# c-f-h/pyiga

Hardware: AMD Instinct MI355X
Metric: assembled elements/sec (3D p=4, 128^3 spans) + HBM-roofline %; 1/2/4/8 GPU (higher is better)
Workload: dtype f64

## Files before the change

### pyiga_amd/csrc/fused3.hip

```cpp
#include "igx_internal.h"
#include "fused_common.h"
#include <algorithm>
#include <cstdio>
#include <cstdlib>
#include <cstring>
#include <vector>

#ifndef BF3_FIXED_PASS
#define BF3_FIXED_PASS 1
#endif
#ifndef BF3_MASS_AXSYM
#define BF3_MASS_AXSYM 1
#endif
#ifndef BF3_MASS_STW
#define BF3_MASS_STW 1
#endif
#ifndef BF3_MASS_STW_QMAX
#define BF3_MASS_STW_QMAX 3
#endif

namespace igx {

template <int P1, int P2, int Q, int NLG, int NRO, int NCW, int SYM> struct BF3Geom {
    static constexpr int P1_ = P1, P2_ = P2, Q_ = Q;
    static constexpr int p1 = P1 - 1, p2 = P2 - 1, W1 = 2 * P1 - 1, W2 = 2 * P2 - 1, TL = 64 * NLG;
    static constexpr int NSET = SYM == 2 ? 2 : 1;
    static constexpr int QS = Q + (Q % 2 == 0 ? 1 : 0), NSP = (TL + Q - 1) / Q;
    static constexpr int TLP = TL + NSP * (QS - Q);
    static constexpr int VS = Q * P2 * 2 + ((Q * P2 * 2) % 4 == 2 ? 0 : 2), NV2 = NSP * VS;
    static constexpr int LS = NRO * TLP + 2;
    static constexpr int NRING = p1 * (p1 + 1) / 2 + p1;
    static constexpr int NRL = NRING + P1;
    static constexpr int T0 = p2 * (p2 + 1) / 2;
    static constexpr int NEL = 2 * p2 * W2;
    static constexpr int off_sets() { return (W1 * LS + 1) & ~1; }
    static constexpr int off_v2(int R) { return (off_sets() + NSET * (NRL * R * W2 + 2) + 1) & ~1; }
    static constexpr int off_etab(int R) { return off_v2(R) + NV2; }
    static constexpr int lds_doubles(int R) { return off_etab(R) + NEL * 2; }
    static constexpr int rmax()
    {
        int R = TL / Q - p2;
        while (R > 1 && lds_doubles(R) * 8 > 160 * 1024) --R;
        return R;
    }
    static constexpr int RMAX = rmax();
    static constexpr int RW = RMAX * W2;
    static constexpr int SETSZ = NRL * RW + 2;
    static constexpr int OFF_PAD = NRL * RW;
    static constexpr int roff(int d) { return RW * ((d - 1) * (d + 2) / 2); }
    static constexpr int OFF_CUR = NRING * RW;
    static constexpr int OFF_SETS = off_sets(), OFF_V2 = off_v2(RMAX), OFF_ETAB = off_etab(RMAX);
    static constexpr int LDS_BYTES = lds_doubles(RMAX) * 8;
    static constexpr int NSUB = (RW + 63) / 64;
    static constexpr int npc(int pl) { return (RMAX + pl - p2 - 1) / (pl - p2); }
    static constexpr int npass(int pl) { return (W1 * npc(pl) + 64 / pl - 1) / (64 / pl); }
    static constexpr int pick()
    {
        int best = 64;
        const int cand[4] = {64, 32, 21, 16};
        for (int i = 1; i < 4; ++i)
            if (cand[i] > 2 * p2 && npass(cand[i]) < npass(best)) best = cand[i];
        return best;
    }
    static constexpr int PL = pick(), PPP = 64 / PL, NPC = npc(PL), RP = PL - p2;
};

struct BF3Blk {
    int i0, j0, diag0, c0i, c0j, cj0, ci0, rlo, rhi, row_lo, nrows, stD, stT, ne;
    long long S12;
};

typedef int bf3_v4i __attribute__((ext_vector_type(4)));

template <class Gm> struct BF3Row {
    int on, l0, c1, rp1d, sub1, sub2, sub3, sub4, sub5;
    __device__ __forceinline__ static BF3Row of(const BFArgs &A, const BF3Blk &B, const int t)
    {
        cip rp1 = (cip)A.rp1, jlo1 = (cip)A.jlo1, jhi1 = (cip)A.jhi1;
        constexpr int p1 = Gm::p1, RW = Gm::RW;
        BF3Row r;
        const int d = t - 1;
        r.on = d >= B.rlo && d < B.rhi;
        const int dc = min(max(d, 0), A.N1 - 1);
        const int jl1 = jlo1[dc];
        r.c1 = jhi1[dc] - jl1; r.l0 = p1 - (dc - jl1);
        r.rp1d = rp1[dc];
        r.sub1 = Gm::roff(1) + (int)((unsigned)dc % 2u) * RW; r.sub2 = Gm::roff(2) + (int)((unsigned)dc % 3u) * RW;
        r.sub3 = Gm::roff(3) + (int)((unsigned)dc % 4u) * RW; r.sub4 = Gm::roff(4) + (int)((unsigned)dc % 5u) * RW;
        r.sub5 = Gm::roff(5) + (int)((unsigned)dc % 6u) * RW;
        return r;
    }
    __device__ __forceinline__ int line_off(const int l) const
    {
        constexpr int p1 = Gm::p1;
        int o = Gm::OFF_CUR + (l - p1) * Gm::RW;
        o = l == p1 - 1 ? sub1 : o;
        if (p1 >= 2) o = l == p1 - 2 ? sub2 : o;
        if (p1 >= 3) o = l == p1 - 3 ? sub3 : o;
        if (p1 >= 4) o = l == p1 - 4 ? sub4 : o;
        if (p1 >= 5) o = l == p1 - 5 ? sub5 : o;
        return o;
    }
    __device__ __forceinline__ bool line_ok(const int l) const { return l < Gm::W1 && l >= l0 && l - l0 < c1; }
};
__device__ __forceinline__ __amdgpu_buffer_rsrc_t bf3_rs(double *ptr, const int len) { return __builtin_amdgcn_make_buffer_rsrc((void *)ptr, (short)0, len, 0x00020000); }

// ... 27 lines not shown
            return;
        }
        const long long shift = (long long)W2 * B.row_lo - Gm::T0;
        const long long lenD = ((long long)B.c0i * B.S12 - shift) * 8, lenT = ((long long)B.c0j * B.S12 - shift) * 8;
        pD = A.data + ((long long)rp0[B.i0] * B.S12 - A.nnz_off + shift); nD = B.stD ? (int)lenD : 0;
        pT = A.data + ((long long)rp0[B.j0] * B.S12 - A.nnz_off + shift); nT = B.stT ? (int)lenT : 0;
        const int c0min = min(B.c0i, B.c0j);
        inv = (int)(max(lenD, lenT) / (8 * max(c0min * 2 - 1, 1))) + 1;
#pragma unroll
        for (int c = 0; c < NSUB; ++c) {
            const int q = c * 64 + lane, rr = q / W2, i2 = B.row_lo + rr;
            const bool ok = q < RW && rr < B.nrows && i2 >= p2 && i2 <= A.N2 - 1 - p2;
            rrv[c] = ok ? W2 * i2 - Gm::T0 : inv;
        }
    }
    __device__ __forceinline__ static int line_of(const int sw, const int c, const int j) { return (int)((unsigned)(sw + ROT * c) % (unsigned)NS) + NS * j; }

    template <int X>
    __device__ __forceinline__ void move_row(double *sets, double *dump, const int sw, const int lane, const Row &r, double *ptr, const int len, const int sK, const int soff0)
    {
        int lb_ = lane, lc_ = lanec;
        asm volatile("" : "+v"(lb_), "+v"(lc_));
        double *bs = sets + X * Gm::SETSZ + lb_, *bc = sets + X * Gm::SETSZ + (NSUB - 1) * 64 + lc_;
        double v[NST];
#pragma unroll
        for (int c = 0; c < NSUB; ++c)
#pragma unroll
            for (int j = 0; j < JMAX; ++j) {
                const int l = line_of(sw, c, j);
                double *src = (c == NSUB - 1 ? bc : bs + c * 64) + r.line_off(min(l, W1 - 1));
// ... 29 lines not shown
            const int sD = 8 * B.c0i * (int)A.S1, sT = 8 * B.c0j * (int)A.S1;
            const int oD = 8 * (W2 * (B.c0i * r.rp1d + B.cj0 * r.c1) - r.l0), oT = 8 * (W2 * (B.c0j * r.rp1d + B.ci0 * r.c1) - r.l0);
            move_row<0>(sets, dump, sw, lane, r, pD, r.on ? nD : 0, sD, oD);
            if (NSET == 2) move_row<1>(sets, dump, sw, lane, r, pT, r.on ? nT : 0, sT, oT);
            if (SYM == 3) move_row<0>(sets, dump, sw, lane, r, pT, r.on ? nT : 0, sT, oT);
            return;
        }
        move_row<0>(sets, dump, sw, lane, r, pD, r.on ? nD : 0, 8 * (B.c0i * r.c1 - 1), 8 * ((int)((long long)B.c0i * A.S2) * r.rp1d + W2 * (B.cj0 * r.c1 - r.l0)));
        if (NSET == 2)
            move_row<1>(sets, dump, sw, lane, r, pT, r.on ? nT : 0, 8 * (B.c0j * r.c1 - 1), 8 * ((int)((long long)B.c0j * A.S2) * r.rp1d + W2 * (B.ci0 * r.c1 - r.l0)));
        if (SYM == 3)
            move_row<0>(sets, dump, sw, lane, r, pT, r.on ? nT : 0, 8 * (B.c0j * r.c1 - 1), 8 * ((int)((long long)B.c0j * A.S2) * r.rp1d + W2 * (B.ci0 * r.c1 - r.l0)));
    }
};

template <int NR, int NLG, int NQ> struct BF3DenseSplit {
    static constexpr int NA = (NR - 2) * NLG, NB = NLG;
    static constexpr int ka() { if (NA == 0) return 0; int k = 1; while (NA * k + NB * ((3 * k + 1) / 2) < NQ) ++k; return k; }
    static constexpr int KA = ka(), KB = NA == 0 ? (NQ + NB - 1) / NB : (3 * KA + 1) / 2;
    static constexpr int QB = NA * KA < NQ ? NA * KA : NQ;
};
constexpr int BF3_FAR = 0x7f000000;
template <class Gm, int NH, int SYM, int K, int QLO, int QHI, int QSTR, bool TR>
struct BF3StoreDense {
    static constexpr int p1 = Gm::p1, p2 = Gm::p2, W1 = Gm::W1, W2 = Gm::W2, WW = W1 * W2, RW = Gm::RW, NSET = SYM == 2 ? 2 : 1;
    using Row = BF3Row<Gm>;
    double svD[K], svT[NSET == 2 ? K : 1];
    int pk[K];
    int lane8;
    double *pD, *pT;
    long long nD, nT;

    __device__ __forceinline__ void init(const BFArgs &A, const BF3Blk &B, const int sw, const int lane)
    {
        cip rp0 = (cip)A.rp0;
        lane8 = lane * 8;
        pD = A.data + ((long long)rp0[B.i0] * B.S12 - A.nnz_off); nD = B.stD ? (long long)B.c0i * B.S12 * 8 : 0;
        pT = A.data + ((long long)rp0[B.j0] * B.S12 - A.nnz_off); nT = B.stT ? (long long)B.c0j * B.S12 * 8 : 0;
#pragma unroll
        for (int k = 0; k < K; ++k) {
            svD[k] = 0.0;
            if (NSET == 2) svT[k] = 0.0;
            const int qi = QLO + sw + QSTR * k;
            const int q = qi * 64 + lane, rr = q / WW, rem = q - rr * WW, l = rem / W2, e = rem - l * W2, i2 = B.row_lo + rr;
            const bool ok = qi < QHI && q < Gm::RMAX * WW && rr < B.nrows && i2 >= p2 && i2 <= A.N2 - 1 - p2;
            pk[k] = ok ? (4 * l) | ((rr * W2 + e) << 6) | (rr << 18) : (int)(0x80000000u | 60u);
        }
// ... 68 lines not shown
        const int lane = lane8 >> 3;
        const int offl = (unsigned)(lane - r.l0) < (unsigned)r.c1 ? 0 : BF3_FAR;
#pragma unroll
        for (int k = 0; k < K; ++k) {
            int pkk = pk[k];
            asm volatile("" : "+v"(pkk));
            const int rr = (pkk >> 18) & 0xff;
            const int q8 = __builtin_amdgcn_ds_bpermute(pkk & 60, offl) + ((QLO + sw + QSTR * k) * 512 + lane8);
            bf2_buffer_store(dD, (int)__mul24(rr, dlD) + q8, 0, svD[k]);
            if (NSET == 2) bf2_buffer_store(dT, (int)__mul24(rr, dlT) + q8, 0, svT[k]);
            if (SYM == 3) bf2_buffer_store(dT, (int)__mul24(rr, dlT) + q8, 0, svD[k]);
        }
    }
};

template <class Gm, int NCW, int NH, int SYM, bool TR>
__device__ __forceinline__ void bf3_edge_rows(const BFArgs &A, const BF3Blk &B, double *sets, const bf3_v4i *etab, const int t, const int cw, const int lane)
{
    constexpr int W1 = Gm::W1, W2 = Gm::W2;
    if (B.ne == 0) return;
    cip rp0 = (cip)A.rp0;
    const BF3Row<Gm> r = BF3Row<Gm>::of(A, B, t);
    const long long shift = (long long)W2 * B.row_lo - Gm::T0;
    static_assert(SYM != 3 || NH == 1, "per-axis symmetry: the second store reads the rows again (no halves, no clears)");
#pragma unroll
    for (int X = 0; X < (SYM == 3 ? 2 : Gm::NSET); ++X) {
        if (X == 0 ? !B.stD : !B.stT) continue;
        const int c0x = X == 0 ? B.c0i : B.c0j, cx = X == 0 ? B.cj0 : B.ci0;
        double *px = A.data + ((long long)rp0[X == 0 ? B.i0 : B.j0] * B.S12 - A.nnz_off + (TR ? 0 : shift));
        const int nx = (int)(((long long)c0x * B.S12 - (TR ? 0 : shift)) * 8);
        const unsigned sA = TR ? (unsigned)(c0x * r.rp1d + cx * r.c1) : (unsigned)(c0x * r.c1);
        const unsigned sC = (unsigned)(8 * c0x * (int)A.S1);
        const int soffr = TR ? 0 : 8 * (int)((long long)c0x * A.S2) * r.rp1d;
        for (int l = (int)((unsigned)(cw + NCW - X) % (unsigned)NCW); l < W1; l += NCW) {
            const unsigned sB = TR ? (unsigned)r.c1 : (unsigned)max(cx * r.c1 + l - r.l0, 0);
            const __amdgpu_buffer_rsrc_t dsc = bf3_rs(px, (r.on && r.line_ok(l)) ? nx : 0);
            double *lb = sets + (SYM == 3 ? 0 : X) * Gm::SETSZ + r.line_off(l);
            for (int ch = 0; ch * 64 < B.ne * W2; ++ch) {
                const bf3_v4i e = etab[min(ch * 64 + lane, Gm::NEL - 1)];
// ... 8 lines not shown
            }
        }
    }
}

struct BF3SweepCtx { const BF3Blk *B; double *sets, *dump; int sw, tlp; };
template <int P1, int Q, int D, int MASK, int RI, int NA, int NLG, class StoreT, bool STW, bool MULT>
__device__ __forceinline__ void bf3_sweeper(const BFArgs &A, const int r0, const int g2l, const int g2, const int s_begin, const int t_sw, const int d_begin,
                                            const int rhi, double *lines, const int LS, const BF3SweepCtx &sc)
{
    constexpr BFRole R = bf_role(MASK, RI);
    constexpr int p1 = P1 - 1;
    constexpr bool ST = STW && (RI >= 1 || bf_nroles(MASK) == 1);
    const int slane = threadIdx.x & 63;
    StoreT store;
    if constexpr (ST) store.init(A, *sc.B, sc.sw, slane);
    BF_STAMP_DECL
    __builtin_amdgcn_s_setprio(BF2_PRIO_S);
    cdp V1 = (cdp)A.V1;
    cip fa1 = (cip)A.fa1;
    double acc[P1][P1];
#pragma unroll
    for (int a = 0; a < P1; ++a)
#pragma unroll
        for (int b = 0; b < P1; ++b) acc[a][b] = 0.0;
    __amdgpu_buffer_rsrc_t rsrc[4][NA];
    int urs[4][NA];
    const int voff = g2 * 8;
#pragma unroll
    for (int t1 = 0; t1 < 4; ++t1)
#pragma unroll
// ... 142 lines not shown
            else bf3_sweeper<P1, Q, D, MASK, RI, NA, NLG, StoreA, STW, MULT>(A, r0, g2l, g2, s_begin, t_sw, d_begin, rhi, lines, LS, sc);
        } else BF3SweepDispatch<P1, Q, D, MASK, NA, NLG, StoreA, StoreB, STW, MULT, RI + 1>::run(A, role, r0, g2l, g2, s_begin, t_sw, d_begin, rhi, lines, LS, sc);
    }
};
template <int P1, int Q, int D, int MASK, int NA, int NLG, class StoreA, class StoreB, bool STW, bool MULT, int RI>
struct BF3SweepDispatch<P1, Q, D, MASK, NA, NLG, StoreA, StoreB, STW, MULT, RI, true> {
    __device__ static __forceinline__ void run(const BFArgs &, int, int, int, int, int, int, int, int, double *, int, const BF3SweepCtx &) {}
};

struct BF3Unit {
    const double *lines, *V2s;
    double *sets;
    int dd, rlo, rhi, nhi, row_lo, nrows, lane, npieces;
    int diag0, stD, stT;
    int rbs1, rbs2, rbs3, rbs4, rbs5;
};
template <class Gm, int NY, int MASK, int SYM, int H>
__device__ __forceinline__ void bf3_unit(const BF3Unit U, const int pass)
{
    constexpr int P2 = Gm::P2_, Q = Gm::Q_, p1 = Gm::p1, p2 = Gm::p2, W1 = Gm::W1, W2 = Gm::W2;
    constexpr int TL = Gm::TL, LS = Gm::LS, RW = Gm::RW, PL = Gm::PL, PPP = Gm::PPP, NPC = Gm::NPC, RP = Gm::RP;
    constexpr int AH = (P2 + 1) / 2;
    constexpr int A0 = H == 2 ? AH : 0, A1 = H == 1 ? AH : P2;
    const int lane = U.lane, dd = U.dd;
    int ln_ = min(lane, PPP * PL - 1);
    asm volatile("" : "+v"(ln_));
    const int ps = ln_ / PL, x = ln_ - ps * PL;
    const int pid = pass * PPP + ps;
    const int k9 = pid / NPC, pj = pid - k9 * NPC;
    const int s1 = pj * RP + x;
// ... 9 lines not shown
        for (int a = 0; a < A1 - A0; ++a)
#pragma unroll
            for (int b = 0; b < P2; ++b) { loc[a][b] = k0 + v0 * (a + 3 * b); asm volatile("" : "+v"(loc[a][b])); }
    }
#else
    bf_element<P2, NY, MASK, A0, A1, Q>(loc, kl, vl, Gm::TLP);
#endif
    const int r3 = s1 - p2;
    const bool item = lane < PPP * PL && pid < U.npieces && x >= p2 && r3 < U.nrows && la < U.nhi;
    const int oshv = max(p2 - (U.row_lo + r3), 0);
    int rb = U.rbs1;
    if (p1 >= 2) rb = la == 2 ? U.rbs2 : rb;
    if (p1 >= 3) rb = la == 3 ? U.rbs3 : rb;
    if (p1 >= 4) rb = la == 4 ? U.rbs4 : rb;
    if (p1 >= 5) rb = la == 5 ? U.rbs5 : rb;
    const int cb = Gm::OFF_CUR + la * RW;
    if (U.stD) {
        double out[W2];
#pragma unroll
        for (int a = A0; a < A1; ++a)
#pragma unroll
            for (int b = 0; b < P2; ++b) {
                if (a == 0) out[b + p2] = loc[0][b];
                else if (a == A0 || b == 0) out[b - a + p2] = bf2_from_lane(((lane - a) & 63) * 4, loc[a - A0][b]);
                else out[b - a + p2] += bf2_from_lane(((lane - a) & 63) * 4, loc[a - A0][b]);
            }
        if (item && row1 >= U.rlo && row1 < U.rhi) {
            double *dste = U.sets + ((colt && la > 0) ? rb : cb) + r3 * W2 - oshv;
            constexpr int OLO = H == 0 ? 0 : p2 - (A1 - 1), OHI = H == 0 ? 2 * p2 : 2 * p2 - A0;
            if (SYM != 0 && U.diag0) {
                const int omax = la == 0 ? p2 : 2 * p2;
#pragma unroll
                for (int o = OLO; o <= OHI; ++o)
                    if (o >= oshv && o <= omax) {
                        if (H == 0) dste[o] = out[o];
                        else (void)__hip_atomic_fetch_add(dste + o, out[o], __ATOMIC_RELAXED, __HIP_MEMORY_SCOPE_WORKGROUP);
                    }
            } else if (H == 0) {
                if (U.row_lo >= p2) {
#pragma unroll
                    for (int o = 0; o < W2; ++o) dste[o] = out[o];
                } else {
#pragma unroll
// ... 15 lines not shown
                            else (void)__hip_atomic_fetch_add(dste + o, out[o], __ATOMIC_RELAXED, __HIP_MEMORY_SCOPE_WORKGROUP);
                        }
                }
            }
        }
    }
    __builtin_amdgcn_sched_barrier(0);
#pragma unroll
    for (int a = 0; a < A1 - A0; ++a)
#pragma unroll
        for (int b = 0; b < P2; ++b) asm volatile("" : "+v"(loc[a][b]));
    __builtin_amdgcn_sched_barrier(0);
#ifdef BF3_NOT
    if (SYM != 0 && U.diag0 && U.stD) {
#else
    if (SYM != 0 && (U.diag0 ? U.stD : U.stT)) {
#endif
        double outT[W2];
#pragma unroll
        for (int b = 0; b < P2; ++b)
#pragma unroll
            for (int a = A0; a < A1; ++a) {
                if (b == 0) outT[a + p2] = loc[a - A0][0];
                else if (a == A0) outT[a + p2 - b] = bf2_from_lane(((lane - b) & 63) * 4, loc[0][b]);
                else outT[a + p2 - b] += bf2_from_lane(((lane - b) & 63) * 4, loc[a - A0][b]);
            }
        if (item && col1 >= U.rlo && col1 < U.rhi) {
            constexpr int ELO = H == 0 ? 0 : A0, EHI = H == 0 ? 2 * p2 : A1 - 1 + p2;
            if (U.diag0) {
                double *dste = U.sets + cb + r3 * W2 - oshv;
                const int emin = la == 0 ? p2 + 1 : oshv;
#pragma unroll
                for (int e = ELO; e <= EHI; ++e)
                    if (e >= emin) {
                        if (H == 0) dste[e] = outT[e];
                        else (void)__hip_atomic_fetch_add(dste + e, outT[e], __ATOMIC_RELAXED, __HIP_MEMORY_SCOPE_WORKGROUP);
                    }
            } else {
                double *dste = U.sets + Gm::SETSZ + (colt ? cb : rb) + r3 * W2 - oshv;
                if (H == 0) {
                    if (U.row_lo >= p2) {
#pragma unroll
                        for (int e = 0; e < W2; ++e) dste[e] = outT[e];
                    } else {
#pragma unroll
                        for (int e = 0; e < W2; ++e)
                            if (e >= oshv) dste[e] = outT[e];
                    }
                } else if (U.row_lo >= p2) {
#pragma unroll
                    for (int e = ELO; e <= EHI; ++e) {
                        if ((H == 1 && e < AH) || (H == 2 && e >= p2 + AH)) dste[e] = outT[e];
                        else (void)__hip_atomic_fetch_add(dste + e, outT[e], __ATOMIC_RELAXED, __HIP_MEMORY_SCOPE_WORKGROUP);
// ... 60 lines not shown
        V2s[sp * Gm::VS + (idx - sp * (Q * P2 * 2))] = (gpt >= 0 && gpt < A.G2) ? A.V2[(long long)win0 * P2 * 2 + idx] : 0.0;
    }
    if (NH >= 2)
        for (int idx = threadIdx.x; idx < Gm::OFF_V2 - Gm::OFF_SETS; idx += blockDim.x) sets[idx] = 0.0;
    const int lo_n = max(0, min(row_hi, min(p2, A.N2)) - row_lo);
    const int hi_s = max(max(p2, A.N2 - p2), row_lo), hi_n = max(0, row_hi - hi_s);
    const int ne = lo_n + hi_n;
    if (threadIdx.x < Gm::NEL) {
        const int k = threadIdx.x / W2, e = threadIdx.x - k * W2;
        bf3_v4i v; v.x = 0; v.y = 0; v.z = 0; v.w = BF2_OOB;
        if (k < ne) {
            const int i2 = k < lo_n ? row_lo + k : hi_s + (k - lo_n);
            const int jl2 = max(i2 - p2, 0), c2 = min(i2 + p2, A.N2 - 1) + 1 - jl2;
            if (e < c2) {
                const int shift = W2 * row_lo - Gm::T0;
                v.x = (i2 - row_lo) * W2 + e; v.y = 8 * A.rp2[i2]; v.z = 8 * c2; v.w = 8 * (e - shift);
                if constexpr (TR) { v.y = 8 * c2; v.z = 8 * e; v.w = A.rp2[i2]; }
            }
        }
        etab[threadIdx.x] = v;
    }

    int task = wave;
    if (NR == 4 && NLG == 2 && NCW == 8) {
        constexpr int tmap[16] = {0, 1, 2, 3, 6, 7, 4, 5, 8, 9, 10, 11, 12, 13, 14, 15};
        task = tmap[wave & 15];
    } else if (NR == 4 && NLG == 3 && NCW == 4) {
        constexpr int tmap[16] = {12, 13, 14, 15, 9, 3, 0, 2, 10, 4, 1, 7, 11, 6, 5, 8};
        task = tmap[wave & 15];
    } else if (NR == 4 && NLG == 2 && NCW == 4) {
        const int sd = wave & 3, k = wave >> 2;
        if (sd < 3) task = k == 0 ? NSW + sd : 2 * (sd + 1) + (k - 1);
        else task = k < 2 ? k : NSW + 3;
    }
    BF3Blk B;
    B.i0 = i0; B.j0 = j0; B.diag0 = diag0; B.c0i = jhi0[i0] - jlo0[i0]; B.c0j = jhi0[j0] - jlo0[j0];
    B.cj0 = j0 - jlo0[i0]; B.ci0 = i0 - jlo0[j0]; B.rlo = rlo; B.rhi = rhi;
    B.row_lo = row_lo; B.nrows = nrows; B.S12 = A.S1 * A.S2; B.ne = ne;
    B.stD = (i0 >= A.own_lo && i0 < A.own_hi) ? 1 : 0;
    B.stT = ((SYM == 2 || SYM == 3) && !diag0 && j0 >= A.own_lo && j0 < A.own_hi) ? 1 : 0;
    constexpr bool STW = NR >= 2 || (SYM == 3 && BF3_MASS_STW && Q <= BF3_MASS_STW_QMAX);
    constexpr int NQ = (Gm::RMAX * W1 * W2 + 63) / 64;
    using Split = BF3DenseSplit<NR < 2 ? 2 : NR, NLG, NQ>;
    using StoreA = BF3StoreDense<Gm, NH, SYM, Split::KA < 1 ? 1 : Split::KA, 0, Split::QB, Split::NA < 1 ? 1 : Split::NA, TR>;
    using StoreB = BF3StoreDense<Gm, NH, SYM, Split::KB, Split::QB, NQ, Split::NB, TR>;
    using StoreC = BF3Store<Gm, NCW, 1, NH, SYM, TR>;
    double *dump = lines + NR * Gm::TLP;
    if (task < NSW) {
        const int role = task / NLG, lg = task % NLG;
        const int g2l = lg * 64 + lane;
        const int g2 = min(max(win0 + g2l, 0), A.G2 - 1);
        const BF3SweepCtx sc{&B, sets, dump, role == NR - 1 ? lg : (role - 1) * NLG + lg, Gm::TLP};
        BF3SweepDispatch<P1, Q, (NH == 3 ? Q / 2 : Q), MASK, NA, NLG, StoreA, StoreB, STW, MULT, 0>::run(A, role, r0, g2l + (g2l / Q) * (Gm::QS - Q), g2, s_begin, t_sw, d_begin, rhi, lines, LS, sc);
        return;
    }

    const int cw = task - NSW;
    BF_STAMP_DECL
    __builtin_amdgcn_s_setprio(BF2_PRIO_C);
    StoreC store;
// ... 1 lines not shown
    const bool cdiag = diag0 || SYM == 3;
    const int nlines = cdiag ? P1 : W1;
    const int npieces = nlines * NPC;
    for (int t = d_begin; t < rhi + 1; ++t) {
        bar_lds();
        const int dd = t - 1;
        BF_SEG_BEGIN();
        if (dd >= d_begin && dd < rhi) {
            BF3Unit U;
            U.lines = lines; U.V2s = V2s; U.sets = sets; U.dd = dd; U.rlo = rlo; U.rhi = rhi; U.row_lo = row_lo; U.nrows = nrows;
            U.nhi = jhi1[dd] - dd;
            U.lane = lane; U.npieces = npieces; U.diag0 = cdiag; U.stD = SYM == 3 ? (B.stD | B.stT) : B.stD; U.stT = B.stT;
            U.rbs1 = Gm::roff(1) + (int)((unsigned)(dd + 1) % 2u) * RW; U.rbs2 = Gm::roff(2) + (int)((unsigned)(dd + 2) % 3u) * RW;
            U.rbs3 = Gm::roff(3) + (int)((unsigned)(dd + 3) % 4u) * RW; U.rbs4 = Gm::roff(4) + (int)((unsigned)(dd + 4) % 5u) * RW;
            U.rbs5 = Gm::roff(5) + (int)((unsigned)(dd + 5) % 6u) * RW;
            const int npass = (npieces + PPP - 1) / PPP;
            const int wslot = (int)((unsigned)(cw + t) % (unsigned)NCW);
            if constexpr (NH == 3) {
                for (int u = wslot; u < 2 * npass; u += NCW) {
                    if (u < npass) bf3_unit<Gm, NY, MASK, SYM, 2>(U, u);
                    else bf3_unit<Gm, NY, MASK, SYM, 1>(U, u - npass);
                }
            } else if (NH == 1 || npass <= NCW) {
                for (int pass = BF3_FIXED_PASS ? cw : wslot; pass < npass; pass += NCW) bf3_unit<Gm, NY, MASK, SYM, 0>(U, pass);
            } else if (BF3_FIXED_PASS && 2 * (npass - NCW) == NCW) {
                bf3_unit<Gm, NY, MASK, SYM, 0>(U, cw);
                if ((cw ^ t) & 1) bf3_unit<Gm, NY, MASK, SYM, 1>(U, NCW + (cw >> 1));
                else bf3_unit<Gm, NY, MASK, SYM, 2>(U, NCW + (cw >> 1));
            } else {
                bf3_unit<Gm, NY, MASK, SYM, 0>(U, wslot);
// ... 30 lines not shown

bool fused3_tr_fits(int p0, int p1, int p2, long long S_mid, long long S_last)
{
    const long long c0max = 2 * p0 + 1, W2 = 2 * p2 + 1;
    (void)p1;
    return 8 * W2 * c0max * S_mid < (1LL << 23) && 2 * S_last + 1 < (1LL << 24) && (2 * S_last + 1) * 8 * c0max * S_mid + 8 * W2 * 16 < (1LL << 32);
}

template <int P1, int P2, int Q, int NY, int MASK, int NA, int NLG, int NCW, int NH, int SYM, bool MULT, bool TR = false>
static int launch_bf3_k(hipStream_t st, const BFArgs &A0, int ncu_ctx)
{
    using Gm = BF3Geom<P1, P2, Q, NLG, bf_nroles(MASK), NCW, SYM>;
    constexpr size_t lds = (size_t)Gm::LDS_BYTES;
    static_assert(lds <= 160 * 1024, "k_bf3: LDS");
    static_assert(Gm::RMAX >= 1 && Gm::RMAX <= 255 && Gm::RW < 4096, "k_bf3: packed slot constants");
    static_assert((bf_nroles(MASK) * NLG + NCW) * 64 <= 1024, "k_bf3: block size");
    static_assert(NCW == 4 || NCW == 8, "k_bf3: contractor waves");
    static_assert(Gm::NSUB * 512 <= 4096, "k_bf3: immediate offsets of the stores");
    static_assert(Gm::NEL <= 1024 && Gm::W1 <= 15, "k_bf3: edge table / line index");
    constexpr int nthreads = (bf_nroles(MASK) * NLG + NCW) * 64;
    const void *fn = (const void *)k_bf3<P1, P2, Q, NY, MASK, NA, NLG, NCW, NH, SYM, MULT, TR>;
    IGX_HIP(hipFuncSetAttribute(fn, hipFuncAttributeMaxDynamicSharedMemorySize, (int)lds));
    int per_cu = 1, ncu = ncu_ctx;
    {
        int occ = 0;
        if (hipOccupancyMaxActiveBlocksPerMultiprocessor(&occ, fn, nthreads, lds) == hipSuccess && occ >= 1) per_cu = occ;
        if (ncu < 1) ncu = 256;
    }
    BFArgs A = A0;
    A.ntiles = (A.N2 + Gm::RMAX - 1) / Gm::RMAX;
// ... 183 lines not shown
```

Baseline: 173.3 million.

## Use a single shared ring set for symmetric off-diagonal blocks in 3D fused assembly

For the SYM==2 path, the kernel now keeps one LDS ring buffer with a wider row stride (2*P2 slots per row) and extra backward rings, in place of two separate ring sets for the block and its transpose. The transposed image is read from the same buffer by new store logic (BF3StoreOne) that uses packed slot indices and ds_bpermute line lookup. A second edge table covers the transposed edge rows. This cuts LDS footprint and the duplicate transpose writes by contractors, which may permit a larger row tile. The cost is more complex indexing, extra ring slots and store-side gather work.

Measured after the change: 164.3 million. 5.2% lower.

```diff
diff --git a/pyiga_amd/csrc/fused3.hip b/pyiga_amd/csrc/fused3.hip
--- a/pyiga_amd/csrc/fused3.hip
+++ b/pyiga_amd/csrc/fused3.hip
@@ -4,6 +4,7 @@
 #include <cstdio>
 #include <cstdlib>
 #include <cstring>
+#include <type_traits>
 #include <vector>
 
 #ifndef BF3_FIXED_PASS
@@ -25,6 +26,8 @@
     static constexpr int P1_ = P1, P2_ = P2, Q_ = Q;
     static constexpr int p1 = P1 - 1, p2 = P2 - 1, W1 = 2 * P1 - 1, W2 = 2 * P2 - 1, TL = 64 * NLG;
     static constexpr int NSET = SYM == 2 ? 2 : 1;
+    static constexpr bool ONE = SYM == 2;
+    static constexpr int EP = ONE ? 2 * P2 : 2 * P2 - 1;
     static constexpr int QS = Q + (Q % 2 == 0 ? 1 : 0), NSP = (TL + Q - 1) / Q;
     static constexpr int TLP = TL + NSP * (QS - Q);
     static constexpr int VS = Q * P2 * 2 + ((Q * P2 * 2) % 4 == 2 ? 0 : 2), NV2 = NSP * VS;
@@ -44,13 +47,19 @@
         return R;
     }
     static constexpr int RMAX = rmax();
-    static constexpr int RW = RMAX * W2;
-    static constexpr int SETSZ = NRL * RW + 2;
-    static constexpr int OFF_PAD = NRL * RW;
+    static constexpr int RW = RMAX * EP;
+    static constexpr int NRL1 = ONE ? 2 * NRING + p1 + 2 : NRL;
+    static constexpr int SETSZ = NRL1 * RW + 2;
+    static constexpr int OFF_PAD = NRL1 * RW;
     static constexpr int roff(int d) { return RW * ((d - 1) * (d + 2) / 2); }
     static constexpr int OFF_CUR = NRING * RW;
-    static constexpr int OFF_SETS = off_sets(), OFF_V2 = off_v2(RMAX), OFF_ETAB = off_etab(RMAX);
-    static constexpr int LDS_BYTES = lds_doubles(RMAX) * 8;
+    static constexpr int OFF_B = (NRING + 2) * RW;
+    static constexpr int roffB(int d) { return OFF_B + RW * ((d - 1) * (d + 4) / 2); }
+    static constexpr int RT = RMAX + 2 * p2;
+    static constexpr int OFF_SETS = off_sets();
+    static constexpr int OFF_V2 = ONE ? (OFF_SETS + SETSZ + 1) & ~1 : off_v2(RMAX);
+    static constexpr int OFF_ETAB = OFF_V2 + NV2;
+    static constexpr int LDS_BYTES = (OFF_ETAB + (ONE ? 2 : 1) * NEL * 2) * 8;
     static constexpr int NSUB = (RW + 63) / 64;
     static constexpr int npc(int pl) { return (RMAX + pl - p2 - 1) / (pl - p2); }
     static constexpr int npass(int pl) { return (W1 * npc(pl) + 64 / pl - 1) / (64 / pl); }
@@ -67,6 +76,7 @@
 
 struct BF3Blk {
     int i0, j0, diag0, c0i, c0j, cj0, ci0, rlo, rhi, row_lo, nrows, stD, stT, ne;
+    int neT;
     long long S12;
 };
 
@@ -74,6 +84,8 @@
 
 template <class Gm> struct BF3Row {
     int on, l0, c1, rp1d, sub1, sub2, sub3, sub4, sub5;
+    int sup1, sup2, sup3, sup4, sup5, cur, curo;
+    int sbb1, sbb2, sbb3, sbb4, sbb5, spb1, spb2, spb3, spb4, spb5;
     __device__ __forceinline__ static BF3Row of(const BFArgs &A, const BF3Blk &B, const int t)
     {
         cip rp1 = (cip)A.rp1, jlo1 = (cip)A.jlo1, jhi1 = (cip)A.jhi1;
@@ -88,8 +100,42 @@
         r.sub1 = Gm::roff(1) + (int)((unsigned)dc % 2u) * RW; r.sub2 = Gm::roff(2) + (int)((unsigned)dc % 3u) * RW;
         r.sub3 = Gm::roff(3) + (int)((unsigned)dc % 4u) * RW; r.sub4 = Gm::roff(4) + (int)((unsigned)dc % 5u) * RW;
         r.sub5 = Gm::roff(5) + (int)((unsigned)dc % 6u) * RW;
+        if constexpr (Gm::ONE) {
+            r.sup1 = Gm::roff(1) + (int)((unsigned)(dc + 1) % 2u) * RW; r.sup2 = Gm::roff(2) + (int)((unsigned)(dc + 2) % 3u) * RW;
+            r.sup3 = Gm::roff(3) + (int)((unsigned)(dc + 3) % 4u) * RW; r.sup4 = Gm::roff(4) + (int)((unsigned)(dc + 4) % 5u) * RW;
+            r.sup5 = Gm::roff(5) + (int)((unsigned)(dc + 5) % 6u) * RW;
+            r.cur = Gm::OFF_CUR + (dc & 1) * RW; r.curo = Gm::OFF_CUR + ((dc & 1) ^ 1) * RW;
+            r.sbb1 = Gm::roffB(1) + (int)((unsigned)dc % 3u) * RW; r.sbb2 = Gm::roffB(2) + (int)((unsigned)dc % 4u) * RW;
+            r.sbb3 = Gm::roffB(3) + (int)((unsigned)dc % 5u) * RW; r.sbb4 = Gm::roffB(4) + (int)((unsigned)dc % 6u) * RW;
+            r.sbb5 = Gm::roffB(5) + (int)((unsigned)dc % 7u) * RW;
+            r.spb1 = Gm::roffB(1) + (int)((unsigned)(dc + 1) % 3u) * RW; r.spb2 = Gm::roffB(2) + (int)((unsigned)(dc + 2) % 4u) * RW;
+            r.spb3 = Gm::roffB(3) + (int)((unsigned)(dc + 3) % 5u) * RW; r.spb4 = Gm::roffB(4) + (int)((unsigned)(dc + 4) % 6u) * RW;
+            r.spb5 = Gm::roffB(5) + (int)((unsigned)(dc + 5) % 7u) * RW;
+        }
         return r;
     }
+    template <class T> __device__ __forceinline__ static int pick5(const T dl, int a1, int a2, int a3, int a4, int a5)
+    {
+        asm("" : "+s"(a1), "+s"(a2), "+s"(a3), "+s"(a4), "+s"(a5));
+        int o = a1;
+        if (Gm::p1 >= 2) o = dl == 2 ? a2 : o;
+        if (Gm::p1 >= 3) o = dl == 3 ? a3 : o;
+        if (Gm::p1 >= 4) o = dl == 4 ? a4 : o;
+        if (Gm::p1 >= 5) o = dl == 5 ? a5 : o;
+        return o;
+    }
+    template <class T> __device__ __forceinline__ int sub_of(const T dl) const { return pick5(dl, sub1, sub2, sub3, sub4, sub5); }
+    template <class T> __device__ __forceinline__ int sup_of(const T dl) const { return pick5(dl, sup1, sup2, sup3, sup4, sup5); }
+    template <class T> __device__ __forceinline__ int subB_of(const T dl) const { return pick5(dl, sbb1, sbb2, sbb3, sbb4, sbb5); }
+    template <class T> __device__ __forceinline__ int supB_of(const T dl) const { return pick5(dl, spb1, spb2, spb3, spb4, spb5); }
+    __device__ __forceinline__ int one_off(const int X, const int l) const
+    {
+        constexpr int p1 = Gm::p1;
+        if (l == p1) return cur;
+        if (X == 0) return l < p1 ? sub_of(p1 - l) : supB_of(l - p1);
+        return l < p1 ? subB_of(p1 - l) : sup_of(l - p1);
+    }
+    __device__ __forceinline__ bool one_clears(const int X, const int l) const { return l < Gm::p1 || (l == Gm::p1 && X == 0); }
     __device__ __forceinline__ int line_off(const int l) const
     {
         constexpr int p1 = Gm::p1;
@@ -147,6 +193,7 @@
             rrv[c] = ok ? W2 * i2 - Gm::T0 : inv;
         }
     }
+    __device__ __forceinline__ void bind(double *, double *) {}
     __device__ __forceinline__ static int line_of(const int sw, const int c, const int j) { return (int)((unsigned)(sw + ROT * c) % (unsigned)NS) + NS * j; }
 
     template <int X>
@@ -206,10 +253,11 @@
     }
 };
 
-template <int NR, int NLG, int NQ> struct BF3DenseSplit {
+template <int NR, int NLG, int NQ, int LN = 3, int LD = 2> struct BF3DenseSplit {
     static constexpr int NA = (NR - 2) * NLG, NB = NLG;
-    static constexpr int ka() { if (NA == 0) return 0; int k = 1; while (NA * k + NB * ((3 * k + 1) / 2) < NQ) ++k; return k; }
-    static constexpr int KA = ka(), KB = NA == 0 ? (NQ + NB - 1) / NB : (3 * KA + 1) / 2;
+    static constexpr int kb(int k) { return (LN * k + LD - 1) / LD; }
+    static constexpr int ka() { if (NA == 0) return 0; int k = 1; while (NA * k + NB * kb(k) < NQ) ++k; return k; }
+    static constexpr int KA = ka(), KB = NA == 0 ? (NQ + NB - 1) / NB : kb(KA);
     static constexpr int QB = NA * KA < NQ ? NA * KA : NQ;
 };
 constexpr int BF3_FAR = 0x7f000000;
@@ -223,6 +271,7 @@
     double *pD, *pT;
     long long nD, nT;
 
+    __device__ __forceinline__ void bind(double *, double *) {}
     __device__ __forceinline__ void init(const BFArgs &A, const BF3Blk &B, const int sw, const int lane)
     {
         cip rp0 = (cip)A.rp0;
@@ -321,15 +370,185 @@
     }
 };
 
+template <class Gm, int NH, int KD, int QLD, int QHD, int KT, int QLT, int QHT, int QSTR, bool TR>
+struct BF3StoreOne {
+    static constexpr int p1 = Gm::p1, p2 = Gm::p2, W1 = Gm::W1, W2 = Gm::W2, WW = W1 * W2, RW = Gm::RW, EP = Gm::EP, RT = Gm::RT;
+    using Row = BF3Row<Gm>;
+    double svD[KD];
+    int pkD[KD], pkT[KT];
+    int lane8;
+    double *pD, *pT, *sets_, *dump_;
+    long long nD, nT;
+
+    __device__ __forceinline__ void bind(double *sets, double *dump) { sets_ = sets; dump_ = dump; }
+    __device__ __forceinline__ void init(const BFArgs &A, const BF3Blk &B, const int sw, const int lane)
+    {
+        cip rp0 = (cip)A.rp0;
+        lane8 = lane * 8;
+        pD = A.data + ((long long)rp0[B.i0] * B.S12 - A.nnz_off); nD = B.stD ? (long long)B.c0i * B.S12 * 8 : 0;
+        pT = A.data + ((long long)rp0[B.j0] * B.S12 - A.nnz_off); nT = B.stT ? (long long)B.c0j * B.S12 * 8 : 0;
+#pragma unroll
+        for (int k = 0; k < KD; ++k) {
+            svD[k] = 0.0;
+            const int qi = QLD + sw + QSTR * k;
+            const int q = qi * 64 + lane, rr = q / WW, rem = q - rr * WW, l = rem / W2, e = rem - l * W2, i2 = B.row_lo + rr;
+            const bool ok = qi < QHD && q < Gm::RMAX * WW && rr < B.nrows && i2 >= p2 && i2 <= A.N2 - 1 - p2;
+            pkD[k] = ok ? (4 * l) | ((rr * EP + e) << 6) | (rr << 18) | (e << 26) : (int)(0x80000000u | 60u);
+        }
+#pragma unroll
+        for (int k = 0; k < KT; ++k) {
+            const int qi = QLT + sw + QSTR * k;
+            const int q = qi * 64 + lane, rr = q / WW, rem = q - rr * WW, l = rem / W2, e = rem - l * W2;
+            const int j2 = B.row_lo - p2 + rr, sr = rr + e - 2 * p2;
+            const bool ok = qi < QHT && q < RT * WW && sr >= 0 && sr < B.nrows && j2 >= p2 && j2 <= A.N2 - 1 - p2;
+            pkT[k] = ok ? (4 * l) | ((sr * EP + 2 * p2 - e) << 6) | (rr << 18) | (e << 26) : (int)(0x80000000u | 60u);
+        }
+    }
+
+    __device__ __forceinline__ static int line_blocks(const Row &r, const int X, const int lane)
+    {
+        const int dlo = p1 - lane, dhi = lane - p1;
+        int lv = X == 0 ? (lane < p1 ? r.sub_of(dlo) : r.supB_of(dhi)) : (lane < p1 ? r.subB_of(dlo) : r.sup_of(dhi));
+        lv = lane == p1 ? r.cur : lv;
+        return lane == 15 ? Gm::OFF_PAD : lv;
+    }
+    __device__ __forceinline__ void fetch(const BFArgs &A, const BF3Blk &B, double *sets, double *dump, const int t, const int sw, const int lane)
+    {
+        const Row r = Row::of(A, B, t);
+        const int lvD = line_blocks(r, 0, lane);
+        const int dcur = r.curo - r.cur;
+#pragma unroll
+        for (int k = 0; k < KD; ++k) {
+            int pkk = pkD[k];
+            asm volatile("" : "+v"(pkk));
+            const int l4 = pkk & 60;
+            double *src = sets + (__builtin_amdgcn_ds_bpermute(l4, lvD) + ((pkk >> 6) & 0xfff));
+            svD[k] = *src;
+#ifndef BF3_NOCLEAR
+            if (NH >= 2) {
+                double *cl = l4 == 4 * p1 ? src + dcur : src;
+                cl = l4 > 4 * p1 ? dump : cl;
+                *cl = 0.0;
+            }
+#endif
+        }
+        (void)sw;
+    }
+
+    __device__ __forceinline__ double take_t(const int pkk, const int lvT) const
+    {
+        const int l4 = pkk & 60;
+        double *src = sets_ + (__builtin_amdgcn_ds_bpermute(l4, lvT) + ((pkk >> 6) & 0xfff));
+        const double v = *src;
+#ifndef BF3_NOCLEAR
+        if (NH >= 2) {
+            double *cl = l4 < 4 * p1 ? src : dump_;
+            *cl = 0.0;
+        }
+#endif
+        return v;
+    }
+    __device__ __forceinline__ void issue(const BFArgs &A, const BF3Blk &B, const int t, const int sw)
+    {
+#ifdef BF3_NOSTORE
+        return;
+#endif
+        const Row r = Row::of(A, B, t);
+        const int lane = lane8 >> 3;
+        const int lvT = line_blocks(r, 1, lane);
+        const long long rowcD = (long long)W2 * B.row_lo - Gm::T0, rowcT = rowcD - (long long)W2 * p2;
+        if constexpr (TR) {
+            const long long shD = (long long)B.c0i * A.S1 * rowcD + (long long)W2 * (B.c0i * r.rp1d + B.cj0 * r.c1) - r.l0;
+            const long long shT = (long long)B.c0j * A.S1 * rowcT + (long long)W2 * (B.c0j * r.rp1d + B.ci0 * r.c1) - r.l0;
+            const __amdgpu_buffer_rsrc_t dD = bf3_rs(pD + shD, r.on ? (int)max(nD - shD * 8, 0LL) : 0);
+            const __amdgpu_buffer_rsrc_t dT = bf3_rs(pT + shT, r.on ? (int)max(nT - shT * 8, 0LL) : 0);
+            const int dlD = 8 * W2 * (B.c0i * (int)A.S1 - r.c1), dlT = 8 * W2 * (B.c0j * (int)A.S1 - r.c1), c18 = 8 * r.c1;
+            const int offl = (unsigned)(lane - r.l0) < (unsigned)r.c1 ? lane8 : BF3_FAR;
+#pragma unroll
+            for (int k = 0; k < KD; ++k) {
+                int pkk = pkD[k];
+                asm volatile("" : "+v"(pkk));
+                const int rr = (pkk >> 18) & 0xff, e = (pkk >> 26) & 15;
+                const int q8 = __builtin_amdgcn_ds_bpermute(pkk & 60, offl) + (int)__mul24(rr * W2 + e, c18);
+                bf2_buffer_store(dD, (int)__mul24(rr, dlD) + q8, 0, svD[k]);
+            }
+#pragma unroll
+            for (int k = 0; k < KT; ++k) {
+                int pkk = pkT[k];
+                asm volatile("" : "+v"(pkk));
+                const int rr = (pkk >> 18) & 0xff, e = (pkk >> 26) & 15;
+                const int q8 = __builtin_amdgcn_ds_bpermute(pkk & 60, offl) + (int)__mul24(rr * W2 + e, c18);
+                bf2_buffer_store(dT, (int)__mul24(rr, dlT) + q8, 0, take_t(pkk, lvT));
+            }
+            return;
+        }
+        const int cD = B.c0i * r.c1, cT = B.c0j * r.c1;
+        const long long shD = (long long)B.c0i * A.S2 * r.rp1d + cD * rowcD + W2 * (B.cj0 * r.c1 - r.l0);
+        const __amdgpu_buffer_rsrc_t dD = bf3_rs(pD + shD, r.on ? (int)max(nD - shD * 8, 0LL) : 0);
+        const int dlD = 8 * W2 * (cD - W1);
+        const long long shT = (long long)B.c0j * A.S2 * r.rp1d + cT * rowcT + W2 * (B.ci0 * r.c1 - r.l0);
+        const __amdgpu_buffer_rsrc_t dT = bf3_rs(pT + shT, r.on ? (int)max(nT - shT * 8, 0LL) : 0);
+        const int dlT = 8 * W2 * (cT - W1);
+        const int offl = (unsigned)(lane - r.l0) < (unsigned)r.c1 ? 0 : BF3_FAR;
+#pragma unroll
+        for (int k = 0; k < KD; ++k) {
+            int pkk = pkD[k];
+            asm volatile("" : "+v"(pkk));
+            const int rr = (pkk >> 18) & 0xff;
+            const int q8 = __builtin_amdgcn_ds_bpermute(pkk & 60, offl) + ((QLD + sw + QSTR * k) * 512 + lane8);
+            bf2_buffer_store(dD, (int)__mul24(rr, dlD) + q8, 0, svD[k]);
+        }
+#pragma unroll
+        for (int k = 0; k < KT; ++k) {
+            int pkk = pkT[k];
+            asm volatile("" : "+v"(pkk));
+            const int rr = (pkk >> 18) & 0xff;
+            const int q8 = __builtin_amdgcn_ds_bpermute(pkk & 60, offl) + ((QLT + sw + QSTR * k) * 512 + lane8);
+            bf2_buffer_store(dT, (int)__mul24(rr, dlT) + q8, 0, take_t(pkk, lvT));
+        }
+    }
+};
+
 template <class Gm, int NCW, int NH, int SYM, bool TR>
 __device__ __forceinline__ void bf3_edge_rows(const BFArgs &A, const BF3Blk &B, double *sets, const bf3_v4i *etab, const int t, const int cw, const int lane)
 {
     constexpr int W1 = Gm::W1, W2 = Gm::W2;
-    if (B.ne == 0) return;
+    if (B.ne == 0 && (!Gm::ONE || B.neT == 0)) return;
     cip rp0 = (cip)A.rp0;
     const BF3Row<Gm> r = BF3Row<Gm>::of(A, B, t);
     const long long shift = (long long)W2 * B.row_lo - Gm::T0;
     static_assert(SYM != 3 || NH == 1, "per-axis symmetry: the second store reads the rows again (no halves, no clears)");
+    if constexpr (Gm::ONE) {
+#pragma unroll
+        for (int X = 0; X < 2; ++X) {
+            const int st = X == 0 ? B.stD : B.stT, nex = X == 0 ? B.ne : B.neT;
+            if (nex == 0 || (NH < 2 && !st)) continue;
+            const int c0x = X == 0 ? B.c0i : B.c0j, cx = X == 0 ? B.cj0 : B.ci0;
+            double *px = A.data + ((long long)rp0[X == 0 ? B.i0 : B.j0] * B.S12 - A.nnz_off + (TR ? 0 : shift));
+            const int nx = st ? (int)(((long long)c0x * B.S12 - (TR ? 0 : shift)) * 8) : 0;
+            const unsigned sA = TR ? (unsigned)(c0x * r.rp1d + cx * r.c1) : (unsigned)(c0x * r.c1);
+            const unsigned sC = (unsigned)(8 * c0x * (int)A.S1);
+            const int soffr = TR ? 0 : 8 * (int)((long long)c0x * A.S2) * r.rp1d;
+            const bf3_v4i *tab = etab + X * Gm::NEL;
+            for (int l = (int)((unsigned)(cw + NCW - X) % (unsigned)NCW); l < W1; l += NCW) {
+                const unsigned sB = TR ? (unsigned)r.c1 : (unsigned)max(cx * r.c1 + l - r.l0, 0);
+                const __amdgpu_buffer_rsrc_t dsc = bf3_rs(px, (r.on && r.line_ok(l)) ? nx : 0);
+                double *lb = sets + r.one_off(X, l), *lc = (X == 0 && l == Gm::p1) ? sets + r.curo : lb;
+                const bool clr = NH >= 2 && r.one_clears(X, l);
+                for (int ch = 0; ch * 64 < nex * W2; ++ch) {
+                    const bf3_v4i e = tab[min(ch * 64 + lane, Gm::NEL - 1)];
+                    const bool ok = ch * 64 + lane < Gm::NEL && e.w != BF2_OOB;
+                    const double v = lb[e.x];
+                    if (clr && ok) lc[e.x] = 0.0;
+                    int off = (int)(__umul24(sA, (unsigned)e.y) + __umul24(sB, (unsigned)e.z));
+                    if constexpr (TR) off += (int)__umul24(sC, (unsigned)e.w) + 8 * (l - r.l0);
+                    else off += e.w;
+                    bf2_buffer_store(dsc, ok ? off : BF2_OOB, soffr, v);
+                }
+            }
+        }
+        return;
+    }
 #pragma unroll
     for (int X = 0; X < (SYM == 3 ? 2 : Gm::NSET); ++X) {
         if (X == 0 ? !B.stD : !B.stT) continue;
@@ -368,7 +587,7 @@
     constexpr bool ST = STW && (RI >= 1 || bf_nroles(MASK) == 1);
     const int slane = threadIdx.x & 63;
     StoreT store;
-    if constexpr (ST) store.init(A, *sc.B, sc.sw, slane);
+    if constexpr (ST) { store.init(A, *sc.B, sc.sw, slane); store.bind(sc.sets, sc.dump); }
     BF_STAMP_DECL
     __builtin_amdgcn_s_setprio(BF2_PRIO_S);
     cdp V1 = (cdp)A.V1;
@@ -541,6 +760,7 @@
     int dd, rlo, rhi, nhi, row_lo, nrows, lane, npieces;
     int diag0, stD, stT;
     int rbs1, rbs2, rbs3, rbs4, rbs5;
+    int rbb1, rbb2, rbb3, rbb4, rbb5;
 };
 template <class Gm, int NY, int MASK, int SYM, int H>
 __device__ __forceinline__ void bf3_unit(const BF3Unit U, const int pass)
@@ -580,8 +800,21 @@
     if (p1 >= 3) rb = la == 3 ? U.rbs3 : rb;
     if (p1 >= 4) rb = la == 4 ? U.rbs4 : rb;
     if (p1 >= 5) rb = la == 5 ? U.rbs5 : rb;
-    const int cb = Gm::OFF_CUR + la * RW;
-    if (U.stD) {
+    constexpr bool ONE = Gm::ONE;
+    constexpr int EP = Gm::EP;
+    const int osh = ONE ? 0 : oshv;
+    const int cb = ONE ? Gm::OFF_CUR + (dd & 1) * RW : Gm::OFF_CUR + la * RW;
+    int ub = cb;
+    if constexpr (ONE) {
+        int rbb = U.rbb1;
+        if (p1 >= 2) rbb = la == 2 ? U.rbb2 : rbb;
+        if (p1 >= 3) rbb = la == 3 ? U.rbb3 : rbb;
+        if (p1 >= 4) rbb = la == 4 ? U.rbb4 : rbb;
+        if (p1 >= 5) rbb = la == 5 ? U.rbb5 : rbb;
+        ub = la == 0 ? cb : rbb;
+    }
+    const bool inD = row1 >= U.rlo && row1 < U.rhi, inT = col1 >= U.rlo && col1 < U.rhi;
+    if (ONE ? (U.stD | U.stT) : U.stD) {
         double out[W2];
 #pragma unroll
         for (int a = A0; a < A1; ++a)
@@ -591,8 +824,8 @@
                 else if (a == A0 || b == 0) out[b - a + p2] = bf2_from_lane(((lane - a) & 63) * 4, loc[a - A0][b]);
                 else out[b - a + p2] += bf2_from_lane(((lane - a) & 63) * 4, loc[a - A0][b]);
             }
-        if (item && row1 >= U.rlo && row1 < U.rhi) {
-            double *dste = U.sets + ((colt && la > 0) ? rb : cb) + r3 * W2 - oshv;
+        if (item && (inD || (ONE && !U.diag0 && inT))) {
+            double *dste = U.sets + (ONE ? (colt ? (la > 0 ? rb : cb) : ub) : ((colt && la > 0) ? rb : cb)) + r3 * EP - osh;
             constexpr int OLO = H == 0 ? 0 : p2 - (A1 - 1), OHI = H == 0 ? 2 * p2 : 2 * p2 - A0;
             if (SYM != 0 && U.diag0) {
                 const int omax = la == 0 ? p2 : 2 * p2;
@@ -638,7 +871,7 @@
 #ifdef BF3_NOT
     if (SYM != 0 && U.diag0 && U.stD) {
 #else
-    if (SYM != 0 && (U.diag0 ? U.stD : U.stT)) {
+    if (SYM != 0 && (U.diag0 ? U.stD : (!ONE && U.stT))) {
 #endif
         double outT[W2];
 #pragma unroll
@@ -649,10 +882,10 @@
                 else if (a == A0) outT[a + p2 - b] = bf2_from_lane(((lane - b) & 63) * 4, loc[0][b]);
                 else outT[a + p2 - b] += bf2_from_lane(((lane - b) & 63) * 4, loc[a - A0][b]);
             }
-        if (item && col1 >= U.rlo && col1 < U.rhi) {
+        if (item && inT) {
             constexpr int ELO = H == 0 ? 0 : A0, EHI = H == 0 ? 2 * p2 : A1 - 1 + p2;
             if (U.diag0) {
-                double *dste = U.sets + cb + r3 * W2 - oshv;
+                double *dste = U.sets + ub + r3 * EP - osh;
                 const int emin = la == 0 ? p2 + 1 : oshv;
 #pragma unroll
                 for (int e = ELO; e <= EHI; ++e)
@@ -660,7 +893,7 @@
                         if (H == 0) dste[e] = outT[e];
                         else (void)__hip_atomic_fetch_add(dste + e, outT[e], __ATOMIC_RELAXED, __HIP_MEMORY_SCOPE_WORKGROUP);
                     }
-            } else {
+            } else if constexpr (!ONE) {
                 double *dste = U.sets + Gm::SETSZ + (colt ? cb : rb) + r3 * W2 - oshv;
                 if (H == 0) {
                     if (U.row_lo >= p2) {
@@ -751,11 +984,32 @@
             const int jl2 = max(i2 - p2, 0), c2 = min(i2 + p2, A.N2 - 1) + 1 - jl2;
             if (e < c2) {
                 const int shift = W2 * row_lo - Gm::T0;
-                v.x = (i2 - row_lo) * W2 + e; v.y = 8 * A.rp2[i2]; v.z = 8 * c2; v.w = 8 * (e - shift);
+                v.x = (i2 - row_lo) * Gm::EP + e + (Gm::ONE ? max(p2 - i2, 0) : 0); v.y = 8 * A.rp2[i2]; v.z = 8 * c2; v.w = 8 * (e - shift);
                 if constexpr (TR) { v.y = 8 * c2; v.z = 8 * e; v.w = A.rp2[i2]; }
             }
         }
         etab[threadIdx.x] = v;
+    }
+    int neT = 0;
+    if constexpr (Gm::ONE) {
+        const int tlo = max(row_lo - p2, 0), thi = min(row_hi + p2, A.N2);
+        const int lo_nT = max(0, min(thi, min(p2, A.N2)) - tlo);
+        const int hi_sT = max(max(p2, A.N2 - p2), tlo), hi_nT = max(0, thi - hi_sT);
+        neT = lo_nT + hi_nT;
+        if (threadIdx.x < Gm::NEL) {
+            const int k = threadIdx.x / W2, e = threadIdx.x - k * W2;
+            bf3_v4i v; v.x = 0; v.y = 0; v.z = 0; v.w = BF2_OOB;
+            if (k < neT) {
+                const int j2 = k < lo_nT ? tlo + k : hi_sT + (k - lo_nT);
+                const int il2 = max(j2 - p2, 0), c2 = min(j2 + p2, A.N2 - 1) + 1 - il2, i2 = il2 + e;
+                if (e < c2 && i2 >= row_lo && i2 < row_hi) {
+                    const int shift = W2 * row_lo - Gm::T0;
+                    v.x = (i2 - row_lo) * Gm::EP + (j2 - i2 + p2); v.y = 8 * A.rp2[j2]; v.z = 8 * c2; v.w = 8 * (e - shift);
+                    if constexpr (TR) { v.y = 8 * c2; v.z = 8 * e; v.w = A.rp2[j2]; }
+                }
+            }
+            etab[Gm::NEL + threadIdx.x] = v;
+        }
     }
 
     int task = wave;
@@ -773,14 +1027,21 @@
     BF3Blk B;
     B.i0 = i0; B.j0 = j0; B.diag0 = diag0; B.c0i = jhi0[i0] - jlo0[i0]; B.c0j = jhi0[j0] - jlo0[j0];
     B.cj0 = j0 - jlo0[i0]; B.ci0 = i0 - jlo0[j0]; B.rlo = rlo; B.rhi = rhi;
-    B.row_lo = row_lo; B.nrows = nrows; B.S12 = A.S1 * A.S2; B.ne = ne;
+    B.row_lo = row_lo; B.nrows = nrows; B.S12 = A.S1 * A.S2; B.ne = ne; B.neT = neT;
     B.stD = (i0 >= A.own_lo && i0 < A.own_hi) ? 1 : 0;
     B.stT = ((SYM == 2 || SYM == 3) && !diag0 && j0 >= A.own_lo && j0 < A.own_hi) ? 1 : 0;
     constexpr bool STW = NR >= 2 || (SYM == 3 && BF3_MASS_STW && Q <= BF3_MASS_STW_QMAX);
     constexpr int NQ = (Gm::RMAX * W1 * W2 + 63) / 64;
     using Split = BF3DenseSplit<NR < 2 ? 2 : NR, NLG, NQ>;
-    using StoreA = BF3StoreDense<Gm, NH, SYM, Split::KA < 1 ? 1 : Split::KA, 0, Split::QB, Split::NA < 1 ? 1 : Split::NA, TR>;
-    using StoreB = BF3StoreDense<Gm, NH, SYM, Split::KB, Split::QB, NQ, Split::NB, TR>;
+    constexpr int NQT = (Gm::RT * W1 * W2 + 63) / 64;
+    using SplitT = BF3DenseSplit<NR < 2 ? 2 : NR, NLG, NQT>;
+    static_assert(!Gm::ONE || STW, "k_bf3: one set of rings needs the store duty on the sweepers");
+    using StoreA1 = BF3StoreOne<Gm, NH, Split::KA < 1 ? 1 : Split::KA, 0, Split::QB, SplitT::KA < 1 ? 1 : SplitT::KA, 0, SplitT::QB, Split::NA < 1 ? 1 : Split::NA, TR>;
+    using StoreB1 = BF3StoreOne<Gm, NH, Split::KB, Split::QB, NQ, SplitT::KB, SplitT::QB, NQT, Split::NB, TR>;
+    using StoreA2 = BF3StoreDense<Gm, NH, SYM, Split::KA < 1 ? 1 : Split::KA, 0, Split::QB, Split::NA < 1 ? 1 : Split::NA, TR>;
+    using StoreB2 = BF3StoreDense<Gm, NH, SYM, Split::KB, Split::QB, NQ, Split::NB, TR>;
+    using StoreA = std::conditional_t<Gm::ONE, StoreA1, StoreA2>;
+    using StoreB = std::conditional_t<Gm::ONE, StoreB1, StoreB2>;
     using StoreC = BF3Store<Gm, NCW, 1, NH, SYM, TR>;
     double *dump = lines + NR * Gm::TLP;
     if (task < NSW) {
@@ -812,6 +1073,11 @@
             U.rbs1 = Gm::roff(1) + (int)((unsigned)(dd + 1) % 2u) * RW; U.rbs2 = Gm::roff(2) + (int)((unsigned)(dd + 2) % 3u) * RW;
             U.rbs3 = Gm::roff(3) + (int)((unsigned)(dd + 3) % 4u) * RW; U.rbs4 = Gm::roff(4) + (int)((unsigned)(dd + 4) % 5u) * RW;
             U.rbs5 = Gm::roff(5) + (int)((unsigned)(dd + 5) % 6u) * RW;
+            if constexpr (Gm::ONE) {
+                U.rbb1 = Gm::roffB(1) + (int)((unsigned)(dd + 1) % 3u) * RW; U.rbb2 = Gm::roffB(2) + (int)((unsigned)(dd + 2) % 4u) * RW;
+                U.rbb3 = Gm::roffB(3) + (int)((unsigned)(dd + 3) % 5u) * RW; U.rbb4 = Gm::roffB(4) + (int)((unsigned)(dd + 4) % 6u) * RW;
+                U.rbb5 = Gm::roffB(5) + (int)((unsigned)(dd + 5) % 7u) * RW;
+            }
             const int npass = (npieces + PPP - 1) / PPP;
             const int wslot = (int)((unsigned)(cw + t) % (unsigned)NCW);
             if constexpr (NH == 3) {
@@ -872,6 +1138,7 @@
     constexpr size_t lds = (size_t)Gm::LDS_BYTES;
     static_assert(lds <= 160 * 1024, "k_bf3: LDS");
     static_assert(Gm::RMAX >= 1 && Gm::RMAX <= 255 && Gm::RW < 4096, "k_bf3: packed slot constants");
+    static_assert(!Gm::ONE || Gm::RT <= 255, "k_bf3: packed slot constants (transposed image)");
     static_assert((bf_nroles(MASK) * NLG + NCW) * 64 <= 1024, "k_bf3: block size");
     static_assert(NCW == 4 || NCW == 8, "k_bf3: contractor waves");
     static_assert(Gm::NSUB * 512 <= 4096, "k_bf3: immediate offsets of the stores");
```
